# fabioiuri/DRecPy

Hardware: AMD Instinct MI355X
Metric: training samples/sec (user-item pairs) (higher is better)
Workload: dtype f32; 1 GPU; CDAE hidden_factors=128 sampled-output sparse-Adagrad on synth-10m-shaped synthetic (10000000 users x 1000000 items, 199573906 positives), corruption 0.2, neg_ratio 5; batch_per_gpu=65536, global_batch=65536, touch_list=prepared ahead on a side stream, batches=fresh device-sampled batch every step (sampler running ahead on the side stream)

## Files before the change

### drecpy_amd/_lib.py

```python
import ctypes as C
import os

_HERE = os.path.dirname(os.path.abspath(__file__))
LIB_PATH = os.path.join(_HERE, 'libdrx.so')

LOSS_BCE, LOSS_MSE = 0, 1
TARGETS_REFERENCE, TARGETS_PER_ROW = 0, 1
OPT_ADAM, OPT_ADAGRAD, OPT_ROWWISE_ADAGRAD = 0, 1, 2
DENSE_AUX_CLEAN = 0x100
KEY_NONE = 0xFFFFFFFF
SHARD_SELF_BYPASS = 1
BATCH_SHARE_USERS = 1


class DrxError(RuntimeError):
    pass


DRX_REC_SIGMOID_BIAS, DRX_REC_BIAS, DRX_REC_CLIP = 0, 1, 2

KNN_METRICS = {'cosine': 0, 'adjusted_cosine': 1, 'cosine_cf': 2, 'jaccard': 3, 'msd': 4, 'pearson': 5}
KNN_USER, KNN_ITEM = 0, 1
KNN_AGGREGATIONS = {'mean': 0, 'weighted_mean': 1}

# ... 109 lines not shown
    'drx_event_synchronize': (C.c_int, [C.c_void_p]),
    'drx_stream_create_cu_slice': (C.c_void_p, [C.c_int32]),
    'drx_stream_destroy': (None, [C.c_void_p]),
    'drx_cdae_forward': (C.c_int, [C.POINTER(CdaeParams), C.POINTER(History), C.POINTER(Batch), C.c_void_p,
                                   C.c_void_p, C.c_void_p]),
    'drx_cdae_scratch_bytes': (C.c_size_t, [C.POINTER(CdaeParams), C.c_int32, C.c_int32, C.c_int32]),
    'drx_cdae_step_dense': (C.c_int, [C.POINTER(CdaeParams), C.POINTER(Optim), C.POINTER(History), C.POINTER(Batch),
                                      C.c_int32, C.c_int32, C.c_void_p, C.c_size_t, C.c_void_p, C.c_void_p]),
    'drx_cdae_step_sparse': (C.c_int, [C.POINTER(CdaeParams), C.POINTER(Optim), C.POINTER(History), C.POINTER(Batch),
                                       C.c_int32, C.c_void_p, C.c_size_t, C.c_void_p, C.c_void_p]),
    'drx_cdae_step_sparse_timed': (C.c_int, [C.POINTER(CdaeParams), C.POINTER(Optim), C.POINTER(History),
                                             C.POINTER(Batch), C.c_int32, C.c_void_p, C.c_size_t, C.c_void_p,
                                             C.POINTER(C.c_void_p), C.c_void_p]),
    'drx_cdae_prep_bytes': (C.c_size_t, [C.POINTER(CdaeParams), C.c_int32, C.c_int32]),
    'drx_cdae_sparse_prepare': (C.c_int, [C.POINTER(CdaeParams), C.POINTER(History), C.POINTER(Batch), C.c_void_p,
                                          C.c_size_t, C.c_void_p]),
    'drx_cdae_step_sparse_prepared': (C.c_int, [C.POINTER(CdaeParams), C.POINTER(Optim), C.POINTER(History),
                                                C.POINTER(Batch), C.c_int32, C.c_void_p, C.c_size_t, C.c_void_p,
                                                C.c_size_t, C.c_void_p, C.POINTER(C.c_void_p), C.c_void_p]),
    'drx_cdae_prep_bytes_hot': (C.c_size_t, [C.POINTER(CdaeParams), C.c_int32, C.c_int32, C.c_int32]),
    'drx_cdae_scratch_bytes_hot': (C.c_size_t, [C.POINTER(CdaeParams), C.c_int32, C.c_int32, C.c_int32]),
    'drx_cdae_sparse_prepare_hot': (C.c_int, [C.POINTER(CdaeParams), C.POINTER(History), C.POINTER(Batch), C.POINTER(HotHead),
                                              C.c_void_p, C.c_size_t, C.c_void_p]),
    'drx_cdae_step_sparse_hot': (C.c_int, [C.POINTER(CdaeParams), C.POINTER(Optim), C.POINTER(History), C.POINTER(Batch),
                                           C.POINTER(HotHead), C.c_int32, C.c_void_p, C.c_size_t, C.c_void_p, C.c_size_t,
                                           C.c_void_p, C.POINTER(C.c_void_p), C.c_void_p]),
    'drx_cdae_hot_rows_for': (C.c_int32, [C.POINTER(CdaeParams), C.c_int32, C.c_int32, C.c_int32, C.c_int32]),
    'drx_cdae_prep_forget': (None, [C.c_void_p]),
    'drx_point_sample_scratch_bytes': (C.c_size_t, [C.c_int32]),
    'drx_list_sample_device': (C.c_int, [C.POINTER(ListGroups), C.c_int32, C.c_int32, C.c_int32, C.c_int32, C.c_uint64, C.c_void_p, C.c_void_p,
                                         C.c_void_p, C.c_void_p]),
    'drx_point_sample': (C.c_int, [C.POINTER(History), C.c_int32, C.c_int32, C.c_int32, C.c_int32, C.c_uint64,
                                   C.c_void_p, C.c_void_p, C.c_void_p, C.c_void_p, C.c_void_p, C.c_size_t, C.c_void_p, C.c_uint32,
                                   C.c_void_p]),
    'drx_point_sample_recorded': (C.c_int, [C.POINTER(History), C.POINTER(History), C.c_int32, C.c_int32, C.c_int32, C.c_int32, C.c_uint64,
                                   C.c_void_p, C.c_void_p, C.c_void_p, C.c_void_p, C.c_void_p, C.c_size_t, C.c_void_p, C.c_uint32,
                                   C.c_void_p]),
    'drx_point_sample_by_user_scratch_bytes': (C.c_size_t, [C.c_int32, C.c_int32]),
    'drx_point_sample_by_user': (C.c_int, [C.POINTER(History), C.POINTER(History), C.c_int32, C.c_int32, C.c_int32, C.c_int32, C.c_uint64,
                                           C.c_void_p, C.c_void_p, C.c_void_p, C.c_void_p, C.c_void_p, C.c_size_t, C.c_void_p, C.c_uint32,
                                           C.c_void_p]),
    'drx_point_sample_valued': (C.c_int, [C.POINTER(History), C.POINTER(History), C.c_void_p, C.c_float, C.c_float, C.c_int32, C.c_int32,
                                          C.c_int32, C.c_int32, C.c_uint64, C.c_void_p, C.c_void_p, C.c_void_p, C.c_void_p]),
    'drx_dmf_distinct_scratch_bytes': (C.c_size_t, [C.c_int32, C.c_int32, C.c_int32]),
    'drx_dmf_batch_distinct_device': (C.c_int, [C.c_void_p, C.c_void_p, C.c_void_p, C.c_int32, C.c_int32, C.c_int32] + [C.c_void_p] * 10 +
                                      [C.c_void_p, C.c_size_t, C.c_void_p]),
# ... 229 lines not shown
```

### drecpy_amd/csrc/drx_cdae.hip

```cpp
#include "drx_common.hpp"
#include "drx_rows.hpp"
#include "drx_segreduce.hpp"
#include <cstring>
#include "drx_scan.hpp"
#include "drx_prep.hpp"
#include "drx_segstream.hpp"
#include "drx_cdae_host.hpp"
#include <type_traits>
#include <mutex>
#include <unordered_map>

#ifdef DRX_STAMPS
static unsigned long long *h_stamps = nullptr;
extern "C" int drx_debug_set_stamps(unsigned long long *buf, unsigned int) { h_stamps = buf; return 0; }
#endif

namespace drx {

struct SparseBufs {
  float *dz1;
  float *g2;
  float *dz2;
  float *lossb;
  float *phead, *ptail;
// ... 910 lines not shown
  (void)hot_layout(c, *p, B, H);
  (void)prep_layout(c, *p, B, n_touch_slots, H);
  return align_up(c.off, 256) + 256;
}

int drx_cdae_sparse_prepare_hot(const DrxCdaeParams *p, const DrxHistory *hist, const DrxBatch *bt, const DrxHotHead *hot,
                                void *prepared, size_t prepared_bytes, void *stream) {
  int rc = check_params(p);
  if (rc) return rc;
  rc = check_batch(hist, bt);
  if (rc || !prepared || !bt->iid || !bt->keep_off || !hot_ok(p, hot)) return DRX_EINVAL;
  Carver cp(prepared, prepared_bytes);
  PrepBufs R = prep_layout(cp, *p, bt->B, bt->n_touch_slots, hot->H);
  if (!cp.ok()) return DRX_ESCRATCH;
  hot_record(prepared, 0);
  rc = prepare_impl(p, hist, bt, R, (hipStream_t)stream, true, TouchPresence{nullptr, WireGeo{1, 0, 1}}, hot->slot, hot->item);
  if (rc) return rc;
  hot_record(prepared, hot->H);
  if (p->ld <= 16) order_by_degree(bt, R, (hipStream_t)stream, true);
  DRX_LAUNCH_CHECK();
  return DRX_OK;
}

int drx_cdae_step_sparse_hot(const DrxCdaeParams *p, const DrxOptim *opt, const DrxHistory *hist, const DrxBatch *bt,
                             const DrxHotHead *hot, int32_t loss_kind, const void *prepared, size_t prepared_bytes, void *scratch,
                             size_t scratch_bytes, float *loss_out, void *const *events, void *stream) {
  if (!hot_ok(p, hot)) return DRX_EINVAL;
  return step_sparse_impl(p, opt, hist, bt, loss_kind, prepared, prepared_bytes, scratch, scratch_bytes, loss_out, events, stream,
                          nullptr, nullptr, hot);
}

int32_t drx_cdae_hot_rows_for(const DrxCdaeParams *p, int32_t opt_kind, int32_t B, int32_t n_touch_slots, int32_t H) {
  if (B < 1 || n_touch_slots < 0 || hot_rows(p, H) <= 0) return 0;
  return hot_head_fits(reduce_form(opt_kind, B, n_touch_slots + 2 * B, *p), p->ld, false, false) ? H : 0;
}

void drx_cdae_prep_forget(const void *prepared) {
  if (prepared) hot_record(prepared, 0);
}

}
```

### drecpy_amd/csrc/drx_common.hpp

```cpp
#pragma once
#include <cstring>
#include <hip/hip_runtime.h>
#include <stdint.h>
#include "drx.h"

#define DRX_HIP(expr)                                  \
  do {                                                 \
    hipError_t e_ = (expr);                            \
    if (e_ != hipSuccess) return (int)e_;              \
  } while (0)

#define DRX_LAUNCH_CHECK()                             \
  do {                                                 \
    hipError_t e_ = hipGetLastError();                 \
    if (e_ != hipSuccess) return (int)e_;              \
  } while (0)

namespace drx {

constexpr int kWave = 64;
constexpr int kBlock = 256;

__host__ __device__ inline uint32_t hash_u32(uint64_t seed, uint32_t a, uint32_t b) {
  uint64_t x = seed + (uint64_t)a * 0x9E3779B97F4A7C15ull + (uint64_t)b * 0xD1B54A32D192ED03ull;
// ... 114 lines not shown
  }
  return m;
}

template <int NT>
__device__ __forceinline__ void degree_counts_body(const int32_t *__restrict__ keep_off, int B, unsigned int *__restrict__ work, int block_id,
                                                   unsigned int *cnt ) {
  for (int i = threadIdx.x; i < 256; i += NT) cnt[i] = 0;
  __syncthreads();
  const int b = block_id * NT + (int)threadIdx.x, lane = threadIdx.x & 63;
  const bool valid = b < B;
  const int d = valid ? degree_bucket(keep_off, b) : 0;
  const unsigned long long m = same_bucket_lanes(valid, d);
  if (valid && lane == __ffsll((long long)m) - 1) atomicAdd(&cnt[d], (unsigned int)__popcll(m));
  __syncthreads();
  for (int i = threadIdx.x; i < 256; i += NT)
    if (cnt[i]) atomicAdd(&work[i], cnt[i]);
}

struct SortRider {
  const int32_t *keep_off;
  int B;
  unsigned int *counts;
};

int sort_pairs_ex(void *temp, size_t temp_bytes, const uint32_t *kin, uint32_t *kout, const uint32_t *vin, uint32_t *vout, size_t n, int end_bit,
                  bool drop_none, hipStream_t stream, bool pre_zeroed = false, SortRider rider = SortRider{nullptr, 0, nullptr});
void sort_pairs_zero_region(void *temp, size_t n, int end_bit, uint32_t **words, size_t *n_words);

inline int bits_for(uint64_t max_key_exclusive) {
  int b = 1;
  while (b < 32 && (1ull << b) < max_key_exclusive) ++b;
  return b;
}

}
```

### drecpy_amd/csrc/drx_prep.hpp

```cpp
#pragma once
#include <algorithm>
#include "drx_common.hpp"
#include "drx_rows.hpp"
#include "drx_segreduce.hpp"
#include "drx_scan.hpp"

namespace drx {

struct WireGeo {
  int ipr, cshift, world;
  __host__ __device__ __forceinline__ uint32_t wire(int item, int is_out) const {
    const int o = item / ipr;
    const uint32_t l = 2u * (uint32_t)(item - o * ipr) + (uint32_t)(is_out ? 1 : 0);
    return (((l >> cshift) * (uint32_t)world + (uint32_t)o) << cshift) | (l & ((1u << cshift) - 1u));
  }
  __host__ __device__ __forceinline__ uint32_t local(uint32_t w) const {
    return (((w >> cshift) / (uint32_t)world) << cshift) | (w & ((1u << cshift) - 1u));
  }
  __host__ __device__ __forceinline__ uint32_t unit(uint32_t w) const { return w >> cshift; }
};

struct TouchPresence {
  uint8_t *present;
  WireGeo G;
// ... 72 lines not shown
    vals[base + jj] = (uint32_t)b;
    if (hs >= 0) atomicOr(&hm[hs], 1u << (b & 15));
    if (pres.present && kf) pres.present[pres.wire(item, 0)] = 1;
  }
  if (lane == 0) {
    const int deg = (int)(e - s);
    keys[base + deg] = (uint32_t)(n_items + bt.iid[b]);       vals[base + deg] = (uint32_t)b;
    if (pres.present) pres.present[pres.wire(bt.iid[b], 1)] = 1;
    keys[base + deg + 1] = (uint32_t)(2 * n_items) + (uint32_t)u;       vals[base + deg + 1] = (uint32_t)b;
  }
  }
  if (hot.slot) {
    __syncthreads();
    uint16_t *const m16 = reinterpret_cast<uint16_t *>(hot.mask);
    const size_t row = 2 * (size_t)hot.Bw;
    const bool tail = blockIdx.x + 1 == gridDim.x && blockIdx.x + 1 < row;
    for (int i = threadIdx.x; i < hot.H; i += kBlock) {
      m16[(size_t)i * row + blockIdx.x] = (uint16_t)hm[i];
      if (tail) m16[(size_t)i * row + blockIdx.x + 1] = 0;
    }
  }
}

static __global__ __launch_bounds__(1024) void k_degree_counts(const int32_t *__restrict__ keep_off, int B, unsigned int *__restrict__ work) {
  __shared__ unsigned int cnt[256];
  degree_counts_body<1024>(keep_off, B, work, (int)blockIdx.x, cnt);
}

template <int NT>
__device__ __forceinline__ void degree_scatter_body(const int32_t *__restrict__ keep_off, int B, unsigned int *__restrict__ work,
                                                    int32_t *__restrict__ order, int block_id, unsigned int *lds ) {
  unsigned int *start = lds, *cnt = lds + 256, *base = lds + 512;
  for (int i = threadIdx.x; i < 256; i += NT) cnt[i] = 0;
  if (threadIdx.x < 64) {
    unsigned int c[4], sum = 0;
#pragma unroll
    for (int q = 0; q < 4; ++q) { c[q] = work[threadIdx.x * 4 + q]; sum += c[q]; }
    unsigned int inc = sum;
#pragma unroll
    for (int o = 1; o < 64; o <<= 1) { const unsigned int t = __shfl_up(inc, o); if ((int)threadIdx.x >= o) inc += t; }
    unsigned int run = inc - sum;
#pragma unroll
    for (int q = 0; q < 4; ++q) { start[threadIdx.x * 4 + q] = run; run += c[q]; }
  }
  __syncthreads();
  const int b = block_id * NT + (int)threadIdx.x, lane = threadIdx.x & 63;
// ... 123 lines not shown

constexpr int kLongBlocks = 256, kShortBlocks = 1024;

struct __attribute__((aligned(32))) WorkItem { int32_t p0, n, user, deg; long long hist_start, pad_; };

struct PrepBufs {
  uint32_t *keys_s, *vals_s, *keys, *vals;
  void *sort_temp;
  size_t sort_bytes;
  uint8_t *solo_v, *solo_o;
  SpanPlan plan;
  int32_t *order;
  int32_t *usamp;
  int32_t *pitem;
  WorkItem *witem;
  int32_t *worder;
  int32_t *n_du;
  unsigned int *order_work;
  int n_chunks;
  size_t result_bytes;
  int T, bits;
  uint32_t *hmask;
  int H, Bw;
};

static inline bool long_segments(int T, const DrxCdaeParams &P) { return (int64_t)T > 8 * ((int64_t)2 * P.n_items + P.n_users); }

#ifndef DRX_STREAM_DEPTH
#define DRX_STREAM_DEPTH 4
#endif
constexpr int kStreamDepth = DRX_STREAM_DEPTH;
constexpr int kStreamIndexBits = 28;
constexpr int kHotMaxG = 32;

enum class ReduceForm { Streamed, PlannedLong, PlannedShort };

template <class Policy> struct PolicyKind;
template <template <int> class PolicyT, int KIND> struct PolicyKind<PolicyT<KIND>> { static constexpr int value = KIND; };
template <int G, int J, class Policy>
constexpr bool kStreamBuilt = kStreamDepth > 0 && J == 1 && G >= 16 && PolicyKind<Policy>::value == DRX_OPT_ADAGRAD;
template <int G, int J, class Policy>
constexpr bool kHotBuilt = kStreamBuilt<G, J, Policy> && G <= kHotMaxG;

static inline ReduceForm reduce_form(int opt_kind, int B, int T, const DrxCdaeParams &K) {
  if (long_segments(T, K)) return ReduceForm::PlannedLong;
  const Geom gm = pick_geom(K.ld);
// ... 37 lines not shown
  R.plan.ext = cv.take<uint8_t>(R.n_chunks);
  {
    R.plan.xstride = (R.n_chunks + 1) / 2;
    const bool placed = long_segments(R.T, P);
    const bool placed_any = placed || DRX_STREAM_PLACED != 0;
    R.plan.xrank = placed_any ? cv.take<uint32_t>((size_t)R.plan.xstride) : nullptr;
    R.plan.xperm = placed_any ? cv.take<uint32_t>((size_t)R.plan.xstride) : nullptr;
    R.usamp = placed ? cv.take<int32_t>(B) : nullptr;
    R.pitem = placed ? cv.take<int32_t>(B) : nullptr;
    R.witem = placed ? cv.take<WorkItem>((size_t)B) : nullptr;
    R.worder = placed ? cv.take<int32_t>(B) : nullptr;
    R.n_du = placed ? cv.take<int32_t>(128) : nullptr;
  }
  R.order = cv.take<int32_t>(B);
  R.result_bytes = align_up(cv.off, 256);
  R.keys = cv.take<uint32_t>(R.T);
  R.vals = cv.take<uint32_t>(R.T);
  R.sort_bytes = sort_pairs_temp_bytes(R.T, R.bits);
  R.sort_temp = cv.take<char>(R.sort_bytes);
  R.order_work = cv.take<unsigned int>(512);
  R.H = H;
  R.Bw = (B + 31) / 32;
  R.hmask = H > 0 ? cv.take<uint32_t>((size_t)H * R.Bw) : nullptr;
  return R;
}

static int plan_zero_words(const PrepBufs &R) { return (int)(((const char *)R.plan.ext + R.n_chunks - (const char *)R.plan.cnt + 3) / 4); }

static int plan_spans(const DrxCdaeParams *p, const DrxBatch *bt, const PrepBufs &R0, hipStream_t st, bool cleared) {
  const PrepBufs &R = R0;
  if (!cleared) DRX_HIP(hipMemsetAsync(R.plan.cnt, 0, (size_t)plan_zero_words(R) * 4, st));
  hipLaunchKernelGGL(k_plan_spans<0>, dim3((R.n_chunks + 255) / 256), dim3(256), 0, st, R.keys_s, R.vals_s, R.T, R.n_chunks,
                     kSegBlock / pick_geom(p->ld).G, bt->B, R.plan);
  if (R.plan.xrank) hipLaunchKernelGGL(k_place_blocks, dim3(256), dim3(256), 0, st, R.plan, R.n_chunks);
  return DRX_OK;
}

static void order_by_degree(const DrxBatch *bt, const PrepBufs &R, hipStream_t st, bool cleared) {
  if (!cleared) (void)hipMemsetAsync(R.order_work, 0, 512 * sizeof(unsigned int), st);
  const int blocks = (bt->B + 1023) / 1024;
  hipLaunchKernelGGL(k_degree_counts, dim3(blocks), dim3(1024), 0, st, bt->keep_off, bt->B, R.order_work);
  hipLaunchKernelGGL(k_degree_scatter, dim3(blocks), dim3(1024), 0, st, bt->keep_off, bt->B, R.order_work, R.order);
}

constexpr int kTpFallback = 0x7fff0001;

// ... 239 lines not shown
  if (share) {
    const int ig = (B + 255) / 256;
    hipLaunchKernelGGL(k_tp_item_flags, dim3(ig), dim3(256), 0, st, ks, B, rt, start, R.pitem, R.n_du);
    rc = scan_i32(sctemp2, scb2, R.pitem, R.pitem, (size_t)B, true, st);
    if (rc) return rc;
    hipLaunchKernelGGL(k_tp_item_finish, dim3(ig), dim3(256), 0, st, ks, vs, B, rt, start, end, hist->indptr, R.usamp, R.pitem, R.witem,
                       R.n_du, R.plan.cnt);
    hipLaunchKernelGGL(k_tp_item_order, dim3(ig), dim3(256), 0, st, ks, B, rt, start, hist->indptr, R.pitem, R.worder, R.n_du);
    hipLaunchKernelGGL((k_tp_count<true>), dim3(egrid), dim3(256), 0, st, *hist, *bt, qthr, U, start, end, vs, cnt, km, rt);
  } else
    hipLaunchKernelGGL((k_tp_count<false>), dim3(egrid), dim3(256), 0, st, *hist, *bt, qthr, U, start, end, vs, cnt, km, rt);
  int *cnt_last = (int *)R.vals;
  DRX_HIP(hipMemcpyAsync(cnt_last, cnt + (nnz - 1), sizeof(int), hipMemcpyDeviceToDevice, st));
  rc = scan_i32(sctemp, scb, cnt, cnt, (size_t)nnz, false, st);
  if (rc) return rc;
  if (share)
    hipLaunchKernelGGL((k_tp_write<true>), dim3(wgrid), dim3(256), 0, st, *hist, *bt, qthr, start, end, vs, cnt, km, R.keys_s, R.vals_s, R.pitem, rt, row_end);
  else
    hipLaunchKernelGGL((k_tp_write<false>), dim3(wgrid), dim3(256), 0, st, *hist, *bt, qthr, start, end, vs, cnt, km, R.keys_s, R.vals_s, R.pitem, rt, row_end);
  hipLaunchKernelGGL(k_tp_tail, dim3(2048), dim3(256), 0, st, ks, vs, B, U, N, cnt + (nnz - 1), cnt_last, R.T, R.keys_s, R.vals_s, R.plan.cnt);
  return DRX_OK;
}

static int prepare_impl(const DrxCdaeParams *p, const DrxHistory *hist, const DrxBatch *bt, const PrepBufs &R, hipStream_t st,
                        bool with_marks = false, TouchPresence pres = TouchPresence{nullptr, WireGeo{1, 0, 1}},
                        const int16_t *hot_slot = nullptr, const int32_t *hot_item = nullptr) {
  const int gpb = kBlock / 16;
  if (R.H > 0 && (!hot_slot || !hot_item || !hot_list_fits(R.T, *p, pres.present != nullptr))) return DRX_EINVAL;
  if (hist->t_rank && hist->t_users && hist->t_pos && hist->t_items && !pres.present && long_segments(R.T, *p)) {
    const int32_t *row_end = nullptr;
    const int rc = prepare_transposed(p, hist, bt, R, st, with_marks, &row_end);
    if (rc == DRX_OK) {
      PrepBufs Rb = R;
      Rb.plan.row_end = row_end;
      Rb.plan.row_end_keys = (uint32_t)p->n_items;
      if (with_marks && p->ld > 16) {
        if (!share_users(p, hist, bt, R)) order_by_degree(bt, R, st, true);
        const int blocks = std::max(2048, (R.n_chunks + 255) / 256);
        hipLaunchKernelGGL(k_plan_and_mark, dim3(blocks), dim3(256), 0, st, R.keys_s, R.vals_s, R.T, R.n_chunks,
                           kSegBlock / pick_geom(p->ld).G, Rb.plan, (uint32_t)p->n_items, bt->B, R.solo_v, R.solo_o, 0, bt->keep_off,
                           R.order_work, R.order);
        if (R.plan.xrank) hipLaunchKernelGGL(k_place_blocks, dim3(256), dim3(256), 0, st, Rb.plan, R.n_chunks);
        return DRX_OK;
      }
      return plan_spans(p, bt, Rb, st, true);
    }
    if (rc != kTpFallback) return rc;
  }
  uint32_t *sort_zero = nullptr;
  size_t sort_zero_words = 0;
  sort_pairs_zero_region(R.sort_temp, (size_t)R.T, R.bits, &sort_zero, &sort_zero_words);
  hipLaunchKernelGGL(k_sparse_touches, dim3((bt->B + gpb - 1) / gpb), dim3(kBlock), hot_table_lds_bytes(R.H), st, p->n_items, *hist, *bt,
                     q_threshold(bt->q), R.keys, R.vals, R.T, R.solo_v, R.plan.cnt, plan_zero_words(R), R.order_work, 512,
                     sort_zero, (int)sort_zero_words, pres, HotMark{R.H > 0 ? hot_slot : nullptr, R.hmask, R.H, R.Bw, hot_item, hot_table_bits(R.H)});
  const bool fused_order = with_marks && p->ld > 16;
  const SortRider rider{fused_order ? bt->keep_off : nullptr, bt->B, R.order_work};
  const int rc = sort_pairs_ex(R.sort_temp, R.sort_bytes, R.keys, R.keys_s, R.vals, R.vals_s, (size_t)R.T, R.bits, true, st, true, rider);
  if (rc) return rc;
  if (with_marks && p->ld > 16) {
    const int blocks = std::max(2048, (R.n_chunks + 255) / 256);
    const int order_blocks = (bt->B + 255) / 256;
    hipLaunchKernelGGL(k_plan_and_mark, dim3(blocks + order_blocks), dim3(256), 0, st, R.keys_s, R.vals_s, R.T, R.n_chunks,
                       kSegBlock / pick_geom(p->ld).G, R.plan, (uint32_t)p->n_items, bt->B, R.solo_v, R.solo_o,
                       order_blocks, bt->keep_off, R.order_work, R.order);
    if (R.plan.xrank) hipLaunchKernelGGL(k_place_blocks, dim3(256), dim3(256), 0, st, R.plan, R.n_chunks);
    return DRX_OK;
  }
  return plan_spans(p, bt, R, st, true);
}

static int mark_solo(const DrxCdaeParams *p, const DrxBatch *bt, const PrepBufs &R, hipStream_t st, bool cleared) {
  if (!cleared) {
    DRX_HIP(hipMemsetAsync(R.solo_v, 0, (size_t)bt->B * 2, st));
  }
  if (p->ld <= 16) return DRX_OK;
  hipLaunchKernelGGL(k_mark_solo, dim3(2048), dim3(256), 0, st, R.keys_s, R.vals_s, R.T, (uint32_t)p->n_items, bt->B, R.solo_v,
                     R.solo_o);
  return DRX_OK;
}
// ... 4 lines not shown
```

### drecpy_amd/csrc/drx_sort.hip

```cpp
#include <cstdlib>
#include <cstring>
#include <hip/hip_runtime.h>
#include "drx_common.hpp"

namespace drx {

#ifndef DRX_SORT_THREADS
#define DRX_SORT_THREADS 512
#endif
#ifndef DRX_SORT_IPT
#define DRX_SORT_IPT 16
#endif
constexpr int kSortThreads = DRX_SORT_THREADS;
constexpr int kSortWaves = kSortThreads / 64;
constexpr int kSortIPT = DRX_SORT_IPT;
constexpr int kSortTile = kSortThreads * kSortIPT;
constexpr int kMaxPasses = 4;
constexpr uint32_t kStAgg = 1u << 30, kStIncl = 2u << 30, kCountMask = (1u << 30) - 1;
constexpr int kDropNone = 1, kFirstPass = 2, kLastPass = 4;

struct SortPlan {
  int passes;
  int rbits[kMaxPasses];
  int shift[kMaxPasses];
// ... 46 lines not shown
    return;
  }
  const size_t hist_threads = (size_t)((int)gridDim.x - rider_blocks) * blockDim.x;
  for (int i = threadIdx.x; i < P.passes * 2048; i += blockDim.x) h[i] = 0;
  __syncthreads();
  const uint32_t lane = threadIdx.x & 63;
  for (size_t i = (size_t)blockIdx.x * blockDim.x + threadIdx.x; i < n; i += hist_threads) {
    const uint32_t k = keys[i];
    if (drop_none && k == DRX_KEY_NONE) continue;
    for (int p = 0; p < P.passes; ++p) {
      const uint32_t rep_bits = 11u - (uint32_t)P.rbits[p];
      const uint32_t d = (k >> P.shift[p]) & ((1u << P.rbits[p]) - 1);
      atomicAdd(&h[p * 2048 + (d << rep_bits) + (lane & ((1u << rep_bits) - 1u))], 1u);
    }
  }
  __syncthreads();
  for (int p = 0; p < P.passes; ++p) {
    const uint32_t rep_bits = 11u - (uint32_t)P.rbits[p], reps = 1u << rep_bits;
    for (uint32_t d = threadIdx.x; d < (1u << P.rbits[p]); d += blockDim.x) {
      uint32_t c = 0;
      for (uint32_t r = 0; r < reps; ++r) c += h[p * 2048 + (d << rep_bits) + r];
      if (c) atomicAdd(&hist[p * 2048 + d], c);
    }
  }
}

template <int R>
__global__ __launch_bounds__(kSortThreads) void k_onesweep_pass(const uint32_t *__restrict__ kin, const uint32_t *__restrict__ vin,
                                                               uint32_t *__restrict__ kout, uint32_t *__restrict__ vout, size_t n, int shift,
                                                               const uint32_t *__restrict__ ghist, uint32_t *ticket, uint32_t *desc, uint32_t n_tiles,
                                                               int flags, uint32_t *next_hist, int next_shift) {
  constexpr int RADIX = 1 << R;
  constexpr int BPT = (RADIX + kSortThreads - 1) / kSortThreads;
  extern __shared__ __align__(16) uint32_t sort_lds[];
  uint32_t (*whist)[RADIX] = reinterpret_cast<uint32_t (*)[RADIX]>(sort_lds);
  uint32_t *gbase = sort_lds + kSortWaves * RADIX;
  uint32_t *lstart = gbase + RADIX;
  uint32_t *skey = lstart + RADIX, *sval = skey + kSortTile;
  constexpr int REPB = 11 - R, REP = 1 << REPB;
  uint32_t *nh = sval + kSortTile;
  __shared__ uint32_t s_tile, s_tile_valid;
  __shared__ uint32_t wl[kSortWaves], wg[kSortWaves];
  const int tid = threadIdx.x, lane = tid & 63, w = tid >> 6;
  const bool drop = flags & kDropNone, first = flags & kFirstPass, last = flags & kLastPass;
  size_t n_valid = n;
  if (drop) {
// ... 180 lines not shown
template <int R>
static int launch_pass(const uint32_t *sk, const uint32_t *sv, uint32_t *dk, uint32_t *dv, size_t n, int shift, const uint32_t *gh, uint32_t *ticket,
                       uint32_t *desc, int tiles, int flags, uint32_t *next_hist, int next_shift, hipStream_t stream) {
  const size_t lds = onesweep_lds_bytes(R);
  if (lds > 48 * 1024) DRX_HIP(hipFuncSetAttribute((const void *)k_onesweep_pass<R>, hipFuncAttributeMaxDynamicSharedMemorySize, (int)lds));
  hipLaunchKernelGGL(k_onesweep_pass<R>, dim3(tiles < sort_grid() ? tiles : sort_grid()), dim3(kSortThreads), lds, stream, sk, sv, dk, dv, n, shift, gh,
                     ticket, desc, (uint32_t)tiles, flags, next_hist, next_shift);
  return 0;
}

size_t sort_pairs_temp_bytes(size_t n, int end_bit) {
  const SortPlan P = sort_plan(end_bit);
  return sort_layout(nullptr, n ? n : 1, P).total + 256;
}

void sort_pairs_zero_region(void *temp, size_t n, int end_bit, uint32_t **words, size_t *n_words) {
  const SortPlan P = sort_plan(end_bit);
  char *t = (char *)align_up((size_t)temp, 256);
  const SortLayout L = sort_layout(t, n ? n : 1, P);
  *words = (uint32_t *)(t + L.zero_begin);
  *n_words = L.zero_bytes / 4;
}

int sort_pairs_ex(void *temp, size_t temp_bytes, const uint32_t *kin, uint32_t *kout, const uint32_t *vin, uint32_t *vout, size_t n, int end_bit,
                  bool drop_none, hipStream_t stream, bool pre_zeroed, SortRider rider) {
  if (n == 0) return 0;
  if (n >= (1u << 30)) return DRX_EINVAL;
  const SortPlan P = sort_plan(end_bit);
  char *t = (char *)align_up((size_t)temp, 256);
  const SortLayout L = sort_layout(t, n, P);
  if ((size_t)(t - (char *)temp) + L.total > temp_bytes) return DRX_ESCRATCH;
  if (!pre_zeroed) DRX_HIP(hipMemsetAsync(t + L.zero_begin, 0, L.zero_bytes, stream));
  int hgrid = (int)((n + 8 * 512 - 1) / (8 * 512));
  if (hgrid > sort_grid()) hgrid = sort_grid();
  SortPlan P1 = P;
  P1.passes = 1;
  const int rider_blocks = rider.keep_off ? (rider.B + 511) / 512 : 0;
  hipLaunchKernelGGL(k_digit_histograms, dim3(hgrid + rider_blocks), dim3(512), 0, stream, kin, n, P1, L.hist, drop_none ? 1 : 0, rider,
                     rider_blocks);
  const uint32_t *src_k = kin, *src_v = vin;
  uint32_t *desc = L.desc;
  for (int p = 0; p < P.passes; ++p) {
    const bool to_out = ((P.passes - 1 - p) & 1) == 0;
    uint32_t *dk = to_out ? kout : L.tmp_k, *dv = to_out ? vout : L.tmp_v;
    const uint32_t *gh = L.hist + (size_t)p * 2048;
    const int flags = (drop_none ? kDropNone : 0) | (p == 0 ? kFirstPass : 0) | (p == P.passes - 1 ? kLastPass : 0);
    int rc;
    uint32_t *nh = p + 1 < P.passes ? L.hist + (size_t)(p + 1) * 2048 : nullptr;
    const int ns = p + 1 < P.passes ? P.shift[p + 1] : 0;
    if (P.rbits[p] == 8) rc = launch_pass<8>(src_k, src_v, dk, dv, n, P.shift[p], gh, L.ticket + p, desc, L.tiles, flags, nh, ns, stream);
    else if (P.rbits[p] == 10) rc = launch_pass<10>(src_k, src_v, dk, dv, n, P.shift[p], gh, L.ticket + p, desc, L.tiles, flags, nh, ns, stream);
    else rc = launch_pass<11>(src_k, src_v, dk, dv, n, P.shift[p], gh, L.ticket + p, desc, L.tiles, flags, nh, ns, stream);
    if (rc) return rc;
    desc += (size_t)L.tiles << P.rbits[p];
    src_k = dk; src_v = dv;
  }
  DRX_LAUNCH_CHECK();
  return 0;
}

int sort_pairs(void *temp, size_t temp_bytes, const uint32_t *kin, uint32_t *kout, const uint32_t *vin,
               uint32_t *vout, size_t n, int end_bit, hipStream_t stream) {
// ... 17 lines not shown
```

### include/drx.h

```cpp
#ifndef DRX_H_
#define DRX_H_

#include <stddef.h>
#include <stdint.h>

#ifdef __cplusplus
extern "C" {
#endif

#define DRX_VERSION 100

enum {
  DRX_OK = 0,
  DRX_EINVAL = -1,
  DRX_ESCRATCH = -2,
  DRX_ENOTIMPL = -3,
  DRX_ERETRY = -4,
  DRX_ECOMM = -5
};

#define DRX_MAX_K 1024
#define DRX_KEY_NONE 0xFFFFFFFFu

enum { DRX_LOSS_BCE = 0, DRX_LOSS_MSE = 1 };
// ... 78 lines not shown

size_t drx_cdae_prep_bytes(const DrxCdaeParams *p, int32_t B, int32_t n_touch_slots);
int drx_cdae_sparse_prepare(const DrxCdaeParams *p, const DrxHistory *hist, const DrxBatch *bt, void *prepared,
                            size_t prepared_bytes, void *stream);
int drx_cdae_step_sparse_prepared(const DrxCdaeParams *p, const DrxOptim *opt, const DrxHistory *hist, const DrxBatch *bt,
                                  int32_t loss_kind, const void *prepared, size_t prepared_bytes, void *scratch,
                                  size_t scratch_bytes, float *loss_out, void *const *events, void *stream);

typedef struct DrxHotHead {
  int32_t H;
  const int16_t *slot;
  const int32_t *item;
} DrxHotHead;
#define DRX_MAX_HOT 1024
size_t drx_cdae_prep_bytes_hot(const DrxCdaeParams *p, int32_t B, int32_t n_touch_slots, int32_t H);
size_t drx_cdae_scratch_bytes_hot(const DrxCdaeParams *p, int32_t B, int32_t n_touch_slots, int32_t H);
int drx_cdae_sparse_prepare_hot(const DrxCdaeParams *p, const DrxHistory *hist, const DrxBatch *bt, const DrxHotHead *hot,
                                void *prepared, size_t prepared_bytes, void *stream);
int drx_cdae_step_sparse_hot(const DrxCdaeParams *p, const DrxOptim *opt, const DrxHistory *hist, const DrxBatch *bt,
                             const DrxHotHead *hot, int32_t loss_kind, const void *prepared, size_t prepared_bytes, void *scratch,
                             size_t scratch_bytes, float *loss_out, void *const *events, void *stream);
int32_t drx_cdae_hot_rows_for(const DrxCdaeParams *p, int32_t opt_kind, int32_t B, int32_t n_touch_slots, int32_t H);
void drx_cdae_prep_forget(const void *prepared);

int drx_batch_offsets(const int64_t *indptr, const int32_t *ids, int32_t B, int32_t *off, void *scratch, size_t scratch_bytes, void *stream);

size_t drx_point_sample_scratch_bytes(int32_t B);
int drx_point_sample(const DrxHistory *hist, int32_t n_users, int32_t n_items, int32_t B, int32_t neg_ratio,
                     uint64_t seed, int32_t *uid, int32_t *iid, float *y, int32_t *keep_off,
                     void *scratch, size_t scratch_bytes, uint64_t *host_mailbox, uint32_t tag, void *stream);
int drx_point_sample_recorded(const DrxHistory *hist, const DrxHistory *recorded, int32_t n_users, int32_t n_items, int32_t B,
                              int32_t neg_ratio, uint64_t seed, int32_t *uid, int32_t *iid, float *y, int32_t *keep_off,
                              void *scratch, size_t scratch_bytes, uint64_t *host_mailbox, uint32_t tag, void *stream);

size_t drx_point_sample_by_user_scratch_bytes(int32_t B, int32_t n_users);
int drx_point_sample_by_user(const DrxHistory *hist, const DrxHistory *recorded, int32_t n_users, int32_t n_items, int32_t B,
                             int32_t neg_ratio, uint64_t seed, int32_t *uid, int32_t *iid, float *y, int32_t *keep_off, void *scratch,
                             size_t scratch_bytes, uint64_t *host_mailbox, uint32_t tag, void *stream);

int drx_point_sample_valued(const DrxHistory *hist, const DrxHistory *recorded, const float *pos_values, float vmin, float vrange,
                            int32_t n_users, int32_t n_items, int32_t B, int32_t neg_ratio, uint64_t seed, int32_t *uid, int32_t *iid,
                            float *y, void *stream);

typedef struct DrxListGroups {
  const int64_t *indptr;
  const int32_t *seq_ids;
// ... 369 lines not shown
```

Measured before the change: 216.1 million samples/s.

## Fuse first sort-digit histogram into touch kernel with persistent grid-stride rounds

Replaces the per-batch-row touch kernel with a grid-capped persistent kernel that loops over rounds, prefetching the next rows' uid, keep_off and indices. While emitting keys it accumulates the low-8-bit digit histogram and degree buckets in LDS and writes per-block partials. The sort then folds these partials instead of running a separate pass over the keys. This removes one full read of the key array and a launch, at the cost of shared-memory atomics in the touch kernel and a partials buffer. A debug export for inspecting the counts is also added.

Result: faster. 219.0 million samples/s, median of 6 (+1.3%).

```diff
diff --git a/drecpy_amd/_lib.py b/drecpy_amd/_lib.py
--- a/drecpy_amd/_lib.py
+++ b/drecpy_amd/_lib.py
@@ -155,6 +155,9 @@
     'drx_cdae_scratch_bytes_hot': (C.c_size_t, [C.POINTER(CdaeParams), C.c_int32, C.c_int32, C.c_int32]),
     'drx_cdae_sparse_prepare_hot': (C.c_int, [C.POINTER(CdaeParams), C.POINTER(History), C.POINTER(Batch), C.POINTER(HotHead),
                                               C.c_void_p, C.c_size_t, C.c_void_p]),
+    'drx_debug_prep_counts': (C.c_int, [C.POINTER(CdaeParams), C.POINTER(History), C.POINTER(Batch), C.POINTER(HotHead), C.c_void_p,
+                                        C.c_int32, C.c_int32, C.c_int32, C.c_void_p, C.c_size_t, C.c_void_p, C.c_void_p, C.c_void_p,
+                                        C.c_void_p, C.c_void_p, C.POINTER(C.c_int32), C.c_void_p]),
     'drx_cdae_step_sparse_hot': (C.c_int, [C.POINTER(CdaeParams), C.POINTER(Optim), C.POINTER(History), C.POINTER(Batch),
                                            C.POINTER(HotHead), C.c_int32, C.c_void_p, C.c_size_t, C.c_void_p, C.c_size_t,
                                            C.c_void_p, C.POINTER(C.c_void_p), C.c_void_p]),
diff --git a/drecpy_amd/csrc/drx_cdae.hip b/drecpy_amd/csrc/drx_cdae.hip
--- a/drecpy_amd/csrc/drx_cdae.hip
+++ b/drecpy_amd/csrc/drx_cdae.hip
@@ -956,6 +956,45 @@
   return DRX_OK;
 }
 
+int drx_debug_prep_counts(const DrxCdaeParams *p, const DrxHistory *hist, const DrxBatch *bt, const DrxHotHead *hot, uint8_t *present,
+                          int32_t ipr, int32_t cshift, int32_t world, void *prepared, size_t prepared_bytes, uint32_t *hist_out,
+                          uint32_t *buckets_out, uint32_t *keys_out, uint32_t *vals_out, uint32_t *mask_out, int32_t *info_out,
+                          void *stream) {
+  int rc = check_params(p);
+  if (rc) return rc;
+  rc = check_batch(hist, bt);
+  if (rc || !prepared || !bt->iid || !bt->keep_off || !hist_out || !buckets_out || !keys_out || !vals_out || !info_out) return DRX_EINVAL;
+  if ((uint64_t)2 * p->n_items + p->n_users + 1 >= 0xFFFFFFFFull) return DRX_EINVAL;
+  if (hot && !hot_ok(p, hot)) return DRX_EINVAL;
+  if (present && (ipr < 1 || cshift < 0 || cshift > 30 || world < 1)) return DRX_EINVAL;
+  const int H = hot ? hot->H : 0;
+  if (H > 0 && !mask_out) return DRX_EINVAL;
+  Carver cp(prepared, prepared_bytes);
+  const PrepBufs R = prep_layout(cp, *p, bt->B, bt->n_touch_slots, H);
+  if (!cp.ok()) return DRX_ESCRATCH;
+  if (H > 0 && !hot_list_fits(R.T, *p, present != nullptr)) return DRX_EINVAL;
+  hipStream_t st = (hipStream_t)stream;
+  hot_record(prepared, 0);
+  launch_touches(p, hist, bt, R, st, TouchPresence{present, WireGeo{present ? ipr : 1, present ? cshift : 0, present ? world : 1}},
+                 H > 0 ? hot->slot : nullptr, H > 0 ? hot->item : nullptr);
+  const SortRider rider{bt->keep_off, bt->B, R.order_work, R.partials, R.partial_rows};
+  const uint32_t *h = nullptr;
+  rc = sort_first_counts(R.sort_temp, R.sort_bytes, R.keys, (size_t)R.T, R.bits, true, st, rider, &h);
+  if (rc) return rc;
+  const int dbits = sort_first_digit_bits(R.bits);
+  DRX_HIP(hipMemcpyAsync(hist_out, h, sizeof(uint32_t) << dbits, hipMemcpyDeviceToDevice, st));
+  DRX_HIP(hipMemcpyAsync(buckets_out, R.order_work, 256 * sizeof(uint32_t), hipMemcpyDeviceToDevice, st));
+  DRX_HIP(hipMemcpyAsync(keys_out, R.keys, (size_t)R.T * sizeof(uint32_t), hipMemcpyDeviceToDevice, st));
+  DRX_HIP(hipMemcpyAsync(vals_out, R.vals, (size_t)R.T * sizeof(uint32_t), hipMemcpyDeviceToDevice, st));
+  if (H > 0) DRX_HIP(hipMemcpyAsync(mask_out, R.hmask, (size_t)H * R.Bw * sizeof(uint32_t), hipMemcpyDeviceToDevice, st));
+  info_out[0] = dbits;
+  info_out[1] = R.partials ? R.partial_rows : 0;
+  info_out[2] = R.T;
+  info_out[3] = DRX_PREP_ROUNDS ? touch_grid(bt->B) : (bt->B + 15) / 16;
+  DRX_LAUNCH_CHECK();
+  return DRX_OK;
+}
+
 int drx_cdae_step_sparse_hot(const DrxCdaeParams *p, const DrxOptim *opt, const DrxHistory *hist, const DrxBatch *bt,
                              const DrxHotHead *hot, int32_t loss_kind, const void *prepared, size_t prepared_bytes, void *scratch,
                              size_t scratch_bytes, float *loss_out, void *const *events, void *stream) {
diff --git a/drecpy_amd/csrc/drx_common.hpp b/drecpy_amd/csrc/drx_common.hpp
--- a/drecpy_amd/csrc/drx_common.hpp
+++ b/drecpy_amd/csrc/drx_common.hpp
@@ -160,11 +160,17 @@
   const int32_t *keep_off;
   int B;
   unsigned int *counts;
+  const uint32_t *partials = nullptr;
+  int partial_rows = 0;
 };
+constexpr int kPartialWords = 512;
+int sort_first_digit_bits(int end_bit);
 
 int sort_pairs_ex(void *temp, size_t temp_bytes, const uint32_t *kin, uint32_t *kout, const uint32_t *vin, uint32_t *vout, size_t n, int end_bit,
                   bool drop_none, hipStream_t stream, bool pre_zeroed = false, SortRider rider = SortRider{nullptr, 0, nullptr});
 void sort_pairs_zero_region(void *temp, size_t n, int end_bit, uint32_t **words, size_t *n_words);
+int sort_first_counts(void *temp, size_t temp_bytes, const uint32_t *kin, size_t n, int end_bit, bool drop_none, hipStream_t stream,
+                      SortRider rider, const uint32_t **hist);
 
 inline int bits_for(uint64_t max_key_exclusive) {
   int b = 1;
diff --git a/drecpy_amd/csrc/drx_prep.hpp b/drecpy_amd/csrc/drx_prep.hpp
--- a/drecpy_amd/csrc/drx_prep.hpp
+++ b/drecpy_amd/csrc/drx_prep.hpp
@@ -118,6 +118,151 @@
   }
 }
 
+#ifndef DRX_PREP_ROUNDS
+#define DRX_PREP_ROUNDS 1
+#endif
+#ifndef DRX_TOUCH_GRID
+#define DRX_TOUCH_GRID 1024
+#endif
+static inline int touch_grid(int B) {
+  const int rounds = (B + kBlock / 16 - 1) / (kBlock / 16);
+  return rounds < DRX_TOUCH_GRID ? rounds : DRX_TOUCH_GRID;
+}
+
+static __global__ __launch_bounds__(kBlock) void k_sparse_touches_rounds(int n_items, DrxHistory H, DrxBatch bt, uint32_t qthr, uint32_t *keys,
+                                                                  uint32_t *vals, int T, uint8_t *solo, uint32_t *zero_a,
+                                                                  int n_zero_a, uint32_t *zero_b, int n_zero_b, uint32_t *zero_c,
+                                                                  int n_zero_c, TouchPresence pres, HotMark hot, uint32_t *part) {
+  constexpr int G = 16, SPR = kBlock / G;
+  const int lane = threadIdx.x % G, grp = threadIdx.x / G;
+  const int B = bt.B, n_rounds = (B + SPR - 1) / SPR, stride = (int)gridDim.x;
+  for (int w = blockIdx.x * kBlock + threadIdx.x; w < n_zero_a; w += gridDim.x * kBlock) zero_a[w] = 0u;
+  for (int w = blockIdx.x * kBlock + threadIdx.x; w < n_zero_b; w += gridDim.x * kBlock) zero_b[w] = 0u;
+  for (int w = blockIdx.x * kBlock + threadIdx.x; w < n_zero_c; w += gridDim.x * kBlock) zero_c[w] = 0u;
+  __shared__ uint32_t hm[DRX_MAX_HOT];
+  __shared__ uint32_t dh[2048];
+  __shared__ uint32_t bh[256];
+  extern __shared__ __align__(16) int hot_table[];
+  const uint32_t tmask = (1u << hot.tbits) - 1u;
+  uint16_t *const hot_slot_of = reinterpret_cast<uint16_t *>(hot_table + tmask + 1);
+  if (part) {
+    for (int i = threadIdx.x; i < 2048; i += kBlock) dh[i] = 0u;
+    for (int i = threadIdx.x; i < 256; i += kBlock) bh[i] = 0u;
+  }
+  if (hot.slot) {
+    for (int i = threadIdx.x; i < hot.H; i += kBlock) hm[i] = 0u;
+    if (DRX_HOT_LDS_LOOKUP) {
+      for (int i = threadIdx.x; i <= (int)tmask; i += kBlock) hot_table[i] = -1;
+      __syncthreads();
+      for (int i = threadIdx.x; i < hot.H; i += kBlock) {
+        const int it = hot.item[i];
+        uint32_t at = hot_table_home(it, hot.tbits);
+        while (atomicCAS(&hot_table[at], -1, it) != -1) at = (at + 1u) & tmask;
+        hot_slot_of[at] = (uint16_t)i;
+      }
+    }
+  }
+  __syncthreads();
+  const uint32_t rep = threadIdx.x & 7u;
+  constexpr int kPre = 2;
+  struct Stage { int u, ko0, ko1, iid; int64_t s, e; };
+  const int S = stride * SPR;
+  int r = (int)blockIdx.x;
+  int b = r * SPR + grp;
+  Stage c{0, 0, 0, 0, 0, 0}, n1 = c;
+  int it[kPre], u2 = 0;
+  if (b < B) { c.u = bt.uid[b]; c.ko0 = bt.keep_off[b]; c.ko1 = bt.keep_off[b + 1]; c.iid = bt.iid[b]; c.s = H.indptr[c.u]; c.e = H.indptr[c.u + 1]; }
+  if (b + S < B) {
+    n1.u = bt.uid[b + S]; n1.ko0 = bt.keep_off[b + S]; n1.ko1 = bt.keep_off[b + S + 1]; n1.iid = bt.iid[b + S];
+    n1.s = H.indptr[n1.u]; n1.e = H.indptr[n1.u + 1];
+  }
+  if (b + 2 * S < B) u2 = bt.uid[b + 2 * S];
+#pragma unroll
+  for (int k = 0; k < kPre; ++k) it[k] = c.s + lane + k * G < c.e ? H.indices[c.s + lane + k * G] : 0;
+  for (; r < n_rounds; r += stride, b += S) {
+    int itn[kPre], u3 = 0;
+    Stage n2{u2, 0, 0, 0, 0, 0};
+#pragma unroll
+    for (int k = 0; k < kPre; ++k) itn[k] = n1.s + lane + k * G < n1.e ? H.indices[n1.s + lane + k * G] : 0;
+    if (b + 2 * S < B) {
+      n2.ko0 = bt.keep_off[b + 2 * S]; n2.ko1 = bt.keep_off[b + 2 * S + 1]; n2.iid = bt.iid[b + 2 * S];
+      n2.s = H.indptr[u2]; n2.e = H.indptr[u2 + 1];
+    }
+    if (b + 3 * S < B) u3 = bt.uid[b + 3 * S];
+    if (b < B) {
+      const int u = c.u, ko0 = c.ko0, ko1 = c.ko1;
+      const int64_t s = c.s, e = c.e;
+      if (solo && lane == 0) { solo[b] = 0; solo[B + b] = 0; }
+      if (b == B - 1)
+        for (int j = ko1 + 2 * B + lane; j < T; j += G) { keys[j] = DRX_KEY_NONE; vals[j] = 0; }
+      const int base = ko0 + 2 * b;
+      const uint8_t *kp = bt.keep ? bt.keep + ko0 : nullptr;
+      auto touch = [&](uint32_t jj, int item) {
+        const bool kf = kp ? (kp[jj] != 0) : (hash_u32(bt.mask_seed, (uint32_t)b, jj) >= qthr);
+        int hs = -1;
+        if (hot.slot && kf) {
+          if (DRX_HOT_LDS_LOOKUP) {
+            for (uint32_t at = hot_table_home(item, hot.tbits);; at = (at + 1u) & tmask) {
+              const int k = hot_table[at];
+              if (k == item) hs = (int)hot_slot_of[at];
+              if (k == item || k == -1) break;
+            }
+          } else hs = (int)hot.slot[item];
+        }
+        const bool listed = kf && hs < 0;
+        keys[base + jj] = listed ? (uint32_t)item : DRX_KEY_NONE;
+        vals[base + jj] = (uint32_t)b;
+        if (part && listed) atomicAdd(&dh[(((uint32_t)item & 255u) << 3) + rep], 1u);
+        if (hs >= 0) atomicOr(&hm[hs], 1u << (b & 15));
+        if (pres.present && kf) pres.present[pres.wire(item, 0)] = 1;
+      };
+#pragma unroll
+      for (int k = 0; k < kPre; ++k)
+        if (s + lane + k * G < e) touch((uint32_t)(lane + k * G), it[k]);
+      for (int64_t j = s + lane + kPre * G; j < e; j += G) touch((uint32_t)(j - s), H.indices[j]);
+      if (lane == 0) {
+        const int deg = (int)(e - s);
+        const uint32_t k_out = (uint32_t)(n_items + c.iid), k_usr = (uint32_t)(2 * n_items) + (uint32_t)u;
+        keys[base + deg] = k_out;       vals[base + deg] = (uint32_t)b;
+        if (pres.present) pres.present[pres.wire(c.iid, 1)] = 1;
+        keys[base + deg + 1] = k_usr;       vals[base + deg + 1] = (uint32_t)b;
+        if (part) {
+          atomicAdd(&dh[((k_out & 255u) << 3) + rep], 1u);
+          atomicAdd(&dh[((k_usr & 255u) << 3) + rep], 1u);
+          const int d = (ko1 - ko0) >> 2;
+          atomicAdd(&bh[255 - (d > 255 ? 255 : d)], 1u);
+        }
+      }
+    }
+    if (hot.slot) {
+      __syncthreads();
+      uint16_t *const m16 = reinterpret_cast<uint16_t *>(hot.mask);
+      const size_t row = 2 * (size_t)hot.Bw;
+      const bool tail = r + 1 == n_rounds && (size_t)r + 1 < row;
+      for (int i = threadIdx.x; i < hot.H; i += kBlock) {
+        m16[(size_t)i * row + r] = (uint16_t)hm[i];
+        if (tail) m16[(size_t)i * row + r + 1] = 0;
+        hm[i] = 0u;
+      }
+      __syncthreads();
+    }
+    c = n1; n1 = n2; u2 = u3;
+#pragma unroll
+    for (int k = 0; k < kPre; ++k) it[k] = itn[k];
+  }
+  if (part) {
+    __syncthreads();
+    uint32_t *const mine = part + (size_t)blockIdx.x * kPartialWords;
+    for (int d = threadIdx.x; d < 256; d += kBlock) {
+      uint32_t c = 0;
+#pragma unroll
+      for (int q = 0; q < 8; ++q) c += dh[(d << 3) + q];
+      mine[d] = c;
+      mine[256 + d] = bh[d];
+    }
+  }
+}
+
 static __global__ __launch_bounds__(1024) void k_degree_counts(const int32_t *__restrict__ keep_off, int B, unsigned int *__restrict__ work) {
   __shared__ unsigned int cnt[256];
   degree_counts_body<1024>(keep_off, B, work, (int)blockIdx.x, cnt);
@@ -287,6 +432,8 @@
   int T, bits;
   uint32_t *hmask;
   int H, Bw;
+  uint32_t *partials;
+  int partial_rows;
 };
 
 static inline bool long_segments(int T, const DrxCdaeParams &P) { return (int64_t)T > 8 * ((int64_t)2 * P.n_items + P.n_users); }
@@ -370,6 +517,8 @@
   R.H = H;
   R.Bw = (B + 31) / 32;
   R.hmask = H > 0 ? cv.take<uint32_t>((size_t)H * R.Bw) : nullptr;
+  R.partial_rows = DRX_PREP_ROUNDS && sort_first_digit_bits(R.bits) == 8 ? touch_grid(B) : 0;
+  R.partials = R.partial_rows > 0 ? cv.take<uint32_t>((size_t)R.partial_rows * kPartialWords) : nullptr;
   return R;
 }
 
@@ -655,10 +804,28 @@
   return DRX_OK;
 }
 
+static void launch_touches(const DrxCdaeParams *p, const DrxHistory *hist, const DrxBatch *bt, const PrepBufs &R, hipStream_t st,
+                           TouchPresence pres, const int16_t *hot_slot, const int32_t *hot_item) {
+  const int gpb = kBlock / 16;
+  (void)gpb;
+  uint32_t *sort_zero = nullptr;
+  size_t sort_zero_words = 0;
+  sort_pairs_zero_region(R.sort_temp, (size_t)R.T, R.bits, &sort_zero, &sort_zero_words);
+  const HotMark hm{R.H > 0 ? hot_slot : nullptr, R.hmask, R.H, R.Bw, hot_item, hot_table_bits(R.H)};
+#if DRX_PREP_ROUNDS
+  hipLaunchKernelGGL(k_sparse_touches_rounds, dim3(touch_grid(bt->B)), dim3(kBlock), hot_table_lds_bytes(R.H), st, p->n_items, *hist, *bt,
+                     q_threshold(bt->q), R.keys, R.vals, R.T, R.solo_v, R.plan.cnt, plan_zero_words(R), R.order_work, 512,
+                     sort_zero, (int)sort_zero_words, pres, hm, R.partials);
+#else
+  hipLaunchKernelGGL(k_sparse_touches, dim3((bt->B + gpb - 1) / gpb), dim3(kBlock), hot_table_lds_bytes(R.H), st, p->n_items, *hist, *bt,
+                     q_threshold(bt->q), R.keys, R.vals, R.T, R.solo_v, R.plan.cnt, plan_zero_words(R), R.order_work, 512,
+                     sort_zero, (int)sort_zero_words, pres, hm);
+#endif
+}
+
 static int prepare_impl(const DrxCdaeParams *p, const DrxHistory *hist, const DrxBatch *bt, const PrepBufs &R, hipStream_t st,
                         bool with_marks = false, TouchPresence pres = TouchPresence{nullptr, WireGeo{1, 0, 1}},
                         const int16_t *hot_slot = nullptr, const int32_t *hot_item = nullptr) {
-  const int gpb = kBlock / 16;
   if (R.H > 0 && (!hot_slot || !hot_item || !hot_list_fits(R.T, *p, pres.present != nullptr))) return DRX_EINVAL;
   if (hist->t_rank && hist->t_users && hist->t_pos && hist->t_items && !pres.present && long_segments(R.T, *p)) {
     const int32_t *row_end = nullptr;
@@ -680,14 +847,9 @@
     }
     if (rc != kTpFallback) return rc;
   }
-  uint32_t *sort_zero = nullptr;
-  size_t sort_zero_words = 0;
-  sort_pairs_zero_region(R.sort_temp, (size_t)R.T, R.bits, &sort_zero, &sort_zero_words);
-  hipLaunchKernelGGL(k_sparse_touches, dim3((bt->B + gpb - 1) / gpb), dim3(kBlock), hot_table_lds_bytes(R.H), st, p->n_items, *hist, *bt,
-                     q_threshold(bt->q), R.keys, R.vals, R.T, R.solo_v, R.plan.cnt, plan_zero_words(R), R.order_work, 512,
-                     sort_zero, (int)sort_zero_words, pres, HotMark{R.H > 0 ? hot_slot : nullptr, R.hmask, R.H, R.Bw, hot_item, hot_table_bits(R.H)});
+  launch_touches(p, hist, bt, R, st, pres, hot_slot, hot_item);
   const bool fused_order = with_marks && p->ld > 16;
-  const SortRider rider{fused_order ? bt->keep_off : nullptr, bt->B, R.order_work};
+  const SortRider rider{fused_order ? bt->keep_off : nullptr, bt->B, R.order_work, R.partials, R.partial_rows};
   const int rc = sort_pairs_ex(R.sort_temp, R.sort_bytes, R.keys, R.keys_s, R.vals, R.vals_s, (size_t)R.T, R.bits, true, st, true, rider);
   if (rc) return rc;
   if (with_marks && p->ld > 16) {
diff --git a/drecpy_amd/csrc/drx_sort.hip b/drecpy_amd/csrc/drx_sort.hip
--- a/drecpy_amd/csrc/drx_sort.hip
+++ b/drecpy_amd/csrc/drx_sort.hip
@@ -92,6 +92,27 @@
       for (uint32_t r = 0; r < reps; ++r) c += h[p * 2048 + (d << rep_bits) + r];
       if (c) atomicAdd(&hist[p * 2048 + d], c);
     }
+  }
+}
+
+constexpr int kFoldCols = 16, kFoldThreads = 256;
+__global__ __launch_bounds__(kFoldThreads) void k_fold_counts(const uint32_t *__restrict__ partials, int rows, uint32_t *__restrict__ hist,
+                                                              unsigned int *__restrict__ counts) {
+  constexpr int RG = kFoldThreads / kFoldCols;
+  __shared__ uint32_t part[RG][kFoldCols];
+  const int col = threadIdx.x % kFoldCols, rg = threadIdx.x / kFoldCols;
+  const int c = (int)blockIdx.x * kFoldCols + col;
+  uint32_t sum = 0;
+#pragma unroll 8
+  for (int r = rg; r < rows; r += RG) sum += partials[(size_t)r * kPartialWords + c];
+  part[rg][col] = sum;
+  __syncthreads();
+  if (rg == 0) {
+    uint32_t tot = 0;
+#pragma unroll
+    for (int q = 0; q < RG; ++q) tot += part[q][col];
+    if (c < 256) hist[c] = tot;
+    else counts[c - 256] += tot;
   }
 }
 
@@ -318,6 +339,41 @@
   *n_words = L.zero_bytes / 4;
 }
 
+int sort_first_digit_bits(int end_bit) { return sort_plan(end_bit).rbits[0]; }
+
+static int launch_first_counts(const SortPlan &P, const SortLayout &L, const uint32_t *kin, size_t n, bool drop_none, const SortRider &rider,
+                               hipStream_t stream) {
+  if (rider.partials) {
+    if (P.rbits[0] != 8 || !drop_none || rider.partial_rows < 1) return DRX_EINVAL;
+    const int cols = rider.keep_off ? kPartialWords : 256;
+    hipLaunchKernelGGL(k_fold_counts, dim3(cols / kFoldCols), dim3(kFoldThreads), 0, stream, rider.partials, rider.partial_rows, L.hist,
+                       rider.counts);
+    return 0;
+  }
+  int hgrid = (int)((n + 8 * 512 - 1) / (8 * 512));
+  if (hgrid > sort_grid()) hgrid = sort_grid();
+  SortPlan P1 = P;
+  P1.passes = 1;
+  const int rider_blocks = rider.keep_off ? (rider.B + 511) / 512 : 0;
+  hipLaunchKernelGGL(k_digit_histograms, dim3(hgrid + rider_blocks), dim3(512), 0, stream, kin, n, P1, L.hist, drop_none ? 1 : 0, rider,
+                     rider_blocks);
+  return 0;
+}
+
+int sort_first_counts(void *temp, size_t temp_bytes, const uint32_t *kin, size_t n, int end_bit, bool drop_none, hipStream_t stream,
+                      SortRider rider, const uint32_t **hist) {
+  if (n == 0 || n >= (1u << 30)) return DRX_EINVAL;
+  const SortPlan P = sort_plan(end_bit);
+  char *t = (char *)align_up((size_t)temp, 256);
+  const SortLayout L = sort_layout(t, n, P);
+  if ((size_t)(t - (char *)temp) + L.total > temp_bytes) return DRX_ESCRATCH;
+  *hist = L.hist;
+  const int rc = launch_first_counts(P, L, kin, n, drop_none, rider, stream);
+  if (rc) return rc;
+  DRX_LAUNCH_CHECK();
+  return 0;
+}
+
 int sort_pairs_ex(void *temp, size_t temp_bytes, const uint32_t *kin, uint32_t *kout, const uint32_t *vin, uint32_t *vout, size_t n, int end_bit,
                   bool drop_none, hipStream_t stream, bool pre_zeroed, SortRider rider) {
   if (n == 0) return 0;
@@ -327,13 +383,8 @@
   const SortLayout L = sort_layout(t, n, P);
   if ((size_t)(t - (char *)temp) + L.total > temp_bytes) return DRX_ESCRATCH;
   if (!pre_zeroed) DRX_HIP(hipMemsetAsync(t + L.zero_begin, 0, L.zero_bytes, stream));
-  int hgrid = (int)((n + 8 * 512 - 1) / (8 * 512));
-  if (hgrid > sort_grid()) hgrid = sort_grid();
-  SortPlan P1 = P;
-  P1.passes = 1;
-  const int rider_blocks = rider.keep_off ? (rider.B + 511) / 512 : 0;
-  hipLaunchKernelGGL(k_digit_histograms, dim3(hgrid + rider_blocks), dim3(512), 0, stream, kin, n, P1, L.hist, drop_none ? 1 : 0, rider,
-                     rider_blocks);
+  const int rc1 = launch_first_counts(P, L, kin, n, drop_none, rider, stream);
+  if (rc1) return rc1;
   const uint32_t *src_k = kin, *src_v = vin;
   uint32_t *desc = L.desc;
   for (int p = 0; p < P.passes; ++p) {
diff --git a/include/drx.h b/include/drx.h
--- a/include/drx.h
+++ b/include/drx.h
@@ -124,6 +124,11 @@
                              size_t scratch_bytes, float *loss_out, void *const *events, void *stream);
 int32_t drx_cdae_hot_rows_for(const DrxCdaeParams *p, int32_t opt_kind, int32_t B, int32_t n_touch_slots, int32_t H);
 void drx_cdae_prep_forget(const void *prepared);
+
+int drx_debug_prep_counts(const DrxCdaeParams *p, const DrxHistory *hist, const DrxBatch *bt, const DrxHotHead *hot, uint8_t *present,
+                          int32_t ipr, int32_t cshift, int32_t world, void *prepared, size_t prepared_bytes, uint32_t *hist_out,
+                          uint32_t *buckets_out, uint32_t *keys_out, uint32_t *vals_out, uint32_t *mask_out, int32_t *info_out,
+                          void *stream);
 
 int drx_batch_offsets(const int64_t *indptr, const int32_t *ids, int32_t B, int32_t *off, void *scratch, size_t scratch_bytes, void *stream);
 
```
